# spcl/EBCC

Measured on AMD Instinct MI355X. Metric: fp32 GB/s encode+decode, 721x1440 ERA5 frames MAX_ERROR=0.5, higher is better.
Workload: dtype f32; 1 GPU; 256-frame batch 721x1440 fp32 per GPU, base_cr=30 MAX_ERROR=0.5 (BASELINE configs[1]); frames_per_gpu=256, parallelism=frames sharded over 1 GPU(s), no collective, hw_queues=4, encode_slices=3

## Files before the change

### ebcc_amd/csrc/engine.hip

```cpp
#include "engine.hpp"

#include <algorithm>
#include <atomic>
#include <cstdarg>
#include <mutex>
#include <string>
#include <type_traits>
#include <cstring>
#include <vector>

#include "../../include/ebcc_hip.h"
#include "search.hpp"

namespace ebcc {

static thread_local std::string g_last_error;

void set_error(const char *fmt, ...)
{
    char buf[512];
    va_list ap;
    va_start(ap, fmt);
    vsnprintf(buf, sizeof buf, fmt, ap);
    va_end(ap);
// ... 583 lines not shown
        EBCC_HIP_CHECK(hipMemcpyAsync(ctx->d_u64b, ctx->h_u64b, n_frames * sizeof(unsigned long long), hipMemcpyHostToDevice, s));
        EBCC_HIP_CHECK(hipMemcpyAsync(ctx->d_active, ctx->h_active, n_frames * sizeof(int), hipMemcpyHostToDevice, s));
        launch_prefix_synthesis_stats(d_data, d_decoded, ctx->rb, (int) n_frames, ctx->d_u64b, ctx->d_active, s);
        fetch_frame_states(ctx, n_frames);
        for (size_t f = 0; f < n_frames; f++) { maxerr_bits[f] = ctx->h_fs[f].maxerr_bits; err_sum[f] = ctx->h_fs[f].err_sum; }
        for (size_t f = 0; f < n_frames; f++) ctx->h_fs[f].exit_above = 0.0f;
        push_frame_states(ctx, n_frames);
        wait_stream(s);
        return 0;
    }
    if (!ensure_cut_slots(ctx, (int) n_probes)) { set_error("ebcc_hip_residual_probe: no cut slots for %zu probes of this grid", n_probes); return 1; }
    const CutSlots &cs = ctx->cut;
    std::vector<FrameState> vfs(n_probes);
    std::vector<unsigned long long> bits(n_probes);
    std::vector<int> on(n_probes), of(n_probes);
    for (size_t v = 0; v < n_probes; v++) {
        bits[v] = cut_bits[v]; on[v] = active[v] ? 1 : 0; of[v] = frame_of[v];
        vfs[v] = ctx->h_fs[frame_of[v]];
        vfs[v].exit_above = exit_above[v];
        vfs[v].maxerr_bits = maxerr_bits[v]; vfs[v].err_sum = err_sum[v];
    }
    EBCC_HIP_CHECK(hipMemcpyAsync(cs.fs, vfs.data(), n_probes * sizeof(FrameState), hipMemcpyHostToDevice, s));
    EBCC_HIP_CHECK(hipMemcpyAsync(cs.bits, bits.data(), n_probes * sizeof(unsigned long long), hipMemcpyHostToDevice, s));
    EBCC_HIP_CHECK(hipMemcpyAsync(cs.active, on.data(), n_probes * sizeof(int), hipMemcpyHostToDevice, s));
    EBCC_HIP_CHECK(hipMemcpyAsync(cs.frame_of, of.data(), n_probes * sizeof(int), hipMemcpyHostToDevice, s));
    launch_prefix_synthesis_slots(d_data, d_decoded, ctx->rb, cs, (int) n_probes, s);
    EBCC_HIP_CHECK(hipMemcpyAsync(vfs.data(), cs.fs, n_probes * sizeof(FrameState), hipMemcpyDeviceToHost, s));
    wait_stream(s);
    for (size_t v = 0; v < n_probes; v++) { maxerr_bits[v] = vfs[v].maxerr_bits; err_sum[v] = vfs[v].err_sum; }
    return 0;
    EBCC_API_CATCH(1)
}

}
int ebcc::check_ims_header(ebcc_hip_ctx *ctx, const uint8_t *b, size_t n, size_t num_bits)
{
    if (n < 15 || b[0] != 'I' || b[1] != 'M' || b[2] != 'S') { set_error("SPIHT stream: bad magic"); return 1; }
    unsigned long long hi = 0;
    for (int i = 0; i < 8; i++) hi = (hi << 8) | b[3 + i];
    unsigned lo = ((unsigned) b[11] << 8) | b[12];
    unsigned stages = (unsigned) (hi >> 58), sx = (unsigned) (hi >> 46) & 0xFFF, sy = (unsigned) (hi >> 34) & 0xFFF;
    unsigned ex = (unsigned) (hi >> 24) & 0x3FF, ey = (unsigned) (hi >> 14) & 0x3FF;
    unsigned long long bits0 = ((hi & 0x1FFF) << 16) | lo;
    const Grid &g = ctx->rb.g;
    if ((int) stages != g.stages || (int) sx != g.size_x || (int) sy != g.size_y || (int) ex != g.extra_x ||
        (int) ey != g.extra_y) {
        set_error("SPIHT stream geometry (%u stages, %ux%u +%u,%u) does not match the context (%dx%d)", stages, sx, sy,
                  ex, ey, g.size_x, g.size_y);
        return 1;
    }
    unsigned long long nb = num_bits > bits0 ? bits0 : num_bits;
    if (nb <= 128) { set_error("SPIHT stream: num_bits must exceed 128"); return 1; }
    return 0;
}
extern "C" {

int ebcc_hip_spiht_decode(ebcc_hip_ctx *ctx, const uint8_t *const *streams, const size_t *sizes,
                          const size_t *num_bits, size_t n_frames, float *d_images_out)
{
    EBCC_API_TRY
    if (check_batch(ctx, n_frames, "ebcc_hip_spiht_decode")) return 1;
    hipStream_t s = ctx->stream;
    const size_t slot = ctx->rb.stream_words * 4;
    for (size_t f = 0; f < n_frames; f++) {
        if (sizes[f] > slot - 64) { set_error("SPIHT stream of %zu bytes exceeds the slot", sizes[f]); return 1; }
        if (check_ims_header(ctx, streams[f], sizes[f], num_bits[f])) return 1;
// ... 16 lines not shown
```

### ebcc_amd/csrc/residual.hpp

```cpp
#pragma once

#include "common.hpp"

namespace ebcc {

struct FrameState {
    unsigned long long min_key, max_key;
    float minv, maxv;
    int has_nonfinite;
    int const_field;
    unsigned long long rmin_key, rmax_key;
    float rmin, rmax;
    double dc_sum;
    float dc;
    int dc_uncertain;
    int cmax;
    int top_step;
    unsigned long long budget;
    unsigned long long emitted;
    unsigned int stream_bytes;
    unsigned int refine_base[32];
    unsigned int refine_count[32];
    unsigned int step_reached[32];
    unsigned int maxerr_bits;
    double err_sum;
    unsigned long long nbad;
    float exit_above;
    int dec_stages, dec_dc, dec_top_step;
    unsigned long long dec_budget;
};

struct ResidualBuffers {
    Grid g;
    int max_frames;
    size_t np;
    float *A, *T;
    int32_t *C;
    int32_t *D, *G;
    uint32_t *lip, *lsp, *lis0, *lis1;
    uint32_t *sigord, *lspidx;
    uint32_t *stream;
    size_t stream_words;
    double *partial;
    FrameState *fs;
};
constexpr int kPartials = 256;

struct CutSlots {
    int capacity = 0;
    size_t stride = 0;
    float *A = nullptr, *T = nullptr, *D = nullptr;
    FrameState *fs = nullptr;
    double *partial = nullptr;
    unsigned long long *bits = nullptr;
    int *active = nullptr;
    int *frame_of = nullptr;
};
bool prefix_slots_supported(const ResidualBuffers &rb, int n_slots);
void launch_slots_setup(const ResidualBuffers &rb, const CutSlots &cs, int n_slots, hipStream_t s);
void launch_prefix_synthesis_slots(const float *data, const float *decoded, const ResidualBuffers &rb, const CutSlots &cs, int n_slots, hipStream_t s);
// ... 48 lines not shown
```

### ebcc_amd/csrc/residual_device.hpp

```cpp
#pragma once

#include "residual.hpp"

namespace ebcc {

__device__ inline float prefix_value_of(uint32_t o, int c, uint32_t slot, unsigned long long B, const unsigned int *rbase, const unsigned int *rreach)
{
    float out = 0.0f;
    if (o != 0xFFFFFFFFu && (unsigned long long) o <= B) {
        const unsigned int a = (unsigned int) (c < 0 ? -c : c);
        const int ss = 31 - __clz(a);
        unsigned int mag = 1u << ss;
        for (int s = ss - 1; s >= 0; --s) {
            if (!rreach[s]) break;
            const unsigned long long ord = (unsigned long long) rbase[s] + slot + 1;
            if (ord > B + 1) break;
            mag |= a & (1u << s);
        }
        out = c < 0 ? -(float) mag : (float) mag;
    }
    return out;
}
__device__ inline float prefix_value(const int32_t *__restrict__ C, const uint32_t *__restrict__ so, const uint32_t *__restrict__ li, size_t i,
                                     unsigned long long B, const unsigned int *rbase, const unsigned int *rreach)
{
    const uint32_t o = so[i];
    if (o == 0xFFFFFFFFu || (unsigned long long) o > B) return 0.0f;
    return prefix_value_of(o, C[i], li[i], B, rbase, rreach);
}

}
```

### ebcc_amd/csrc/residual_dwt.hip

```cpp
#include <cstring>
#include <cmath>
#include <mutex>
#include "residual.hpp"
#include "residual_device.hpp"
#include "j2k.hpp"

namespace ebcc {

namespace {

__device__ constexpr float kAlpha = -1.586134342f;
__device__ constexpr float kBeta  = -0.05298011854f;
__device__ constexpr float kGamma = 0.8829110762f;
__device__ constexpr float kDelta = 0.44355068522f;
__device__ constexpr float kXi    = 1.149604398f;

constexpr int kRowThreads = 256;
constexpr int kColThreads = 1024;

template <typename Idx>
__device__ inline void lift_forward_tile(float *E, float *O, int half, int lines, Idx at, int tid, int nt)
{
    const int total = half * lines;
    for (int i = tid; i < total; i += nt) {
        int k = i / lines, l = i - k * lines;
        float o = O[at(k, l)];
        if (k + 1 < half) o = o + kAlpha * (E[at(k, l)] + E[at(k + 1, l)]);
        else              o = o + (2 * kAlpha) * E[at(k, l)];
        O[at(k, l)] = o;
    }
    __syncthreads();
    for (int i = tid; i < total; i += nt) {
        int k = i / lines, l = i - k * lines;
        float e = E[at(k, l)];
        if (k > 0) e = e + kBeta * (O[at(k, l)] + O[at(k - 1, l)]);
// ... 345 lines not shown
    {
        const float E0 = div_xi(Ein), O0 = Oin * kXi;
        int k = j - 1;
        float e1 = 0;
        if (k >= 0 && k < half) e1 = E_1 - kDelta * (O_1 + (k > 0 ? O_2 : O0));
        k = j - 2;
        float o1 = 0;
        if (k >= 0 && k < half) o1 = O_2 - kGamma * (a1 + (k + 1 < half ? e1 : a2));
        k = j - 3;
        float e2 = 0;
        if (k >= 0 && k < half) e2 = a2 - kBeta * (b1 + (k > 0 ? b2 : o1));
        k = j - 4;
        x_even = c1;
        x_odd = (k + 1 < half) ? b2 - kAlpha * (c1 + e2) : b2 - (2 * kAlpha) * c1;
        O_2 = O_1; O_1 = O0; E_1 = E0;
        a2 = a1; a1 = e1;
        b2 = b1; b1 = o1;
        c1 = e2;
    }
    __device__ void interior(float Ein, float Oin, float &x_even, float &x_odd)
    {
        const float E0 = div_xi(Ein), O0 = Oin * kXi;
        const float e1 = E_1 - kDelta * (O_1 + O_2);
        const float o1 = O_2 - kGamma * (a1 + e1);
        const float e2 = a2 - kBeta * (b1 + b2);
        x_even = c1;
        x_odd = b2 - kAlpha * (c1 + e2);
        O_2 = O_1; O_1 = O0; E_1 = E0;
        a2 = a1; a1 = e1;
        b2 = b1; b1 = o1;
        c1 = e2;
    }
};

constexpr int kStreamT = 128;
__global__ __launch_bounds__(kStreamT) void k_cols_inv_stream(const float *__restrict__ src, float *__restrict__ dst, Grid g, size_t np,
                                                               const int32_t *__restrict__ Cb, const uint32_t *__restrict__ sigordb,
                                                               const uint32_t *__restrict__ lspidxb, const FrameState *fsb,
                                                               const unsigned long long *trunc_bits, const int *active)
{
    const int frame = blockIdx.y;
    if (active && !active[frame]) return;
    const FrameState &fs = fsb[frame];
    unsigned long long nb = trunc_bits[frame], bits0 = fs.budget + 128;
    if (nb > bits0) nb = bits0;
    const unsigned long long B = nb - 128;
    __shared__ unsigned int rbase[32], rreach[32];
    if (threadIdx.x < 32) { rbase[threadIdx.x] = fs.refine_base[threadIdx.x]; rreach[threadIdx.x] = fs.step_reached[threadIdx.x]; }
    __syncthreads();
    const int nx = g.nx, ny = g.ny, half = ny >> 1, hx = nx >> 1;
    const int col = blockIdx.x * kStreamT + threadIdx.x;
    if (col >= nx) return;
    const float *a = src + (size_t) frame * np;
    float *out = dst + (size_t) frame * np;
    const int32_t *C = Cb + (size_t) frame * np;
    const uint32_t *so = sigordb + (size_t) frame * np, *li = lspidxb + (size_t) frame * np;
    const int per = (half + (int) gridDim.z - 1) / (int) gridDim.z, ka = (int) blockIdx.z * per, kb = min(half, ka + per);
    const int jstart = max(ka - 2, 0);
    struct Raw { float ll; uint32_t eo, el; int ec; uint32_t oo, ol; int oc; };
    const bool left = col < hx;
    auto fetch = [&](int j, Raw &r) {
        const int jj = min(j, half - 1);
        const size_t ie = (size_t) jj * nx + col, io = (size_t) (half + jj) * nx + col;
        r.ll = left ? a[ie] : 0.0f;
        r.eo = left ? 0xFFFFFFFFu : so[ie]; r.ec = 0; r.el = 0;
        if (r.eo != 0xFFFFFFFFu && (unsigned long long) r.eo <= B) { r.ec = C[ie]; r.el = li[ie]; }
        r.oo = so[io]; r.oc = 0; r.ol = 0;
        if (r.oo != 0xFFFFFFFFu && (unsigned long long) r.oo <= B) { r.oc = C[io]; r.ol = li[io]; }
    };
    auto value = [&](const Raw &r, float &e, float &o) {
        e = left ? r.ll : prefix_value_of(r.eo, r.ec, r.el, B, rbase, rreach);
        o = prefix_value_of(r.oo, r.oc, r.ol, B, rbase, rreach);
    };
    RPipe p;
    Raw cur;
    fetch(jstart, cur);
    for (int j = jstart; j < kb + 4; j++) {
        Raw nxt;
        fetch(j + 1, nxt);
        float e_in, o_in, xe, xo;
        value(cur, e_in, o_in);
        p.step(j, half, e_in, o_in, xe, xo);
        const int k = j - 4;
        if (k >= ka && k < kb) {
            out[(size_t) (2 * k) * nx + col] = xe;
            out[(size_t) (2 * k + 1) * nx + col] = xo;
        }
        cur = nxt;
    }
}

constexpr int kFusePairs = 60;
constexpr int kFuseMaxWaves = 16;
__global__ __launch_bounds__(64 * kFuseMaxWaves) void k_finest_inv_use(const float *__restrict__ src, Grid g, size_t np, const int32_t *__restrict__ Cb,
                                                        const uint32_t *__restrict__ sigordb, const uint32_t *__restrict__ lspidxb,
                                                        const unsigned long long *trunc_bits, const int *active, RowUse u, int strips, int n_frames, int pieces,
                                                        const int *frame_of, size_t src_stride)
{
    struct { int strip, frame, piece; } tb{(int) blockIdx.x * ((int) blockDim.x >> 6) + ((int) threadIdx.x >> 6), (int) blockIdx.y % n_frames, (int) blockIdx.y / n_frames};
    const int slot = tb.frame;
    if (active && !active[slot]) return;
    const int frame = frame_of ? frame_of[slot] : slot;
    const FrameState &fs = u.fs[slot];
    unsigned long long nb = trunc_bits[slot], bits0 = fs.budget + 128;
    if (nb > bits0) nb = bits0;
    const unsigned long long B = nb - 128;
    __shared__ unsigned int rbase[32], rreach[32];
    if (threadIdx.x < 32) { rbase[threadIdx.x] = fs.refine_base[threadIdx.x]; rreach[threadIdx.x] = fs.step_reached[threadIdx.x]; }
    __syncthreads();
    if (tb.strip >= strips) return;
    const int lane = (int) threadIdx.x & 63;
    const int nx = g.nx, ny = g.ny, half = ny >> 1, hx = nx >> 1;
    const int k = tb.strip * kFusePairs + lane - 2;
    const bool in_range = k >= 0 && k < hx;
    const bool owner = lane >= 2 && lane < 2 + kFusePairs && in_range;
    const int kc = min(max(k, 0), hx - 1);
    const float *a = src + (size_t) slot * src_stride;
    const int32_t *C = Cb + (size_t) frame * np;
    const uint32_t *so = sigordb + (size_t) frame * np, *li = lspidxb + (size_t) frame * np;
    const float *x = u.data + (size_t) frame * u.n_pix, *d = u.decoded + (size_t) frame * u.n_pix;
    const float dc = fs.dc, rmin = fs.rmin, rng = fs.rmax - fs.rmin;
    const int per = (half + pieces - 1) / pieces, ka = tb.piece * per, kb = min(half, ka + per);
    const size_t part = (size_t) slot * kPartials + (size_t) (tb.strip + strips * tb.piece);
    const int jstart = max(ka - 2, 0);
    const float exit_above = fs.exit_above;
    if (exit_above > 0.0f && __uint_as_float(__hip_atomic_load(&u.fs[slot].maxerr_bits, __ATOMIC_RELAXED, __HIP_MEMORY_SCOPE_AGENT)) > exit_above) {
        if (lane == 0) u.partial[part] = 0.0;
        return;
    }
    struct Det { uint32_t o, l; int c; };
    struct Raw { float ll; Det lh, hl, hh; };
    auto det = [&](size_t i, Det &t) {
        t.o = so[i]; t.c = 0; t.l = 0;
        if (t.o != 0xFFFFFFFFu && (unsigned long long) t.o <= B) { t.c = C[i]; t.l = li[i]; }
    };
    auto fetch = [&](int j, Raw &r) {
        const int jj = min(j, half - 1);
        const size_t top = (size_t) jj * nx, bot = (size_t) (half + jj) * nx;
        r.ll = a[top + kc];
        det(bot + kc, r.lh);
        det(top + hx + kc, r.hl);
        det(bot + hx + kc, r.hh);
    };
    auto val = [&](const Det &t) { return prefix_value_of(t.o, t.c, t.l, B, rbase, rreach); };
    const bool first = !(k > 0), last = !(k + 1 < hx);
    auto hsynth = [&](float e_raw, float o_raw, float &even, float &odd) {
        const float E0 = div_xi(e_raw), O0 = o_raw * kXi;
        const float Ol = lane_below(O0), Or = lane_above(O0);
        const float e1 = E0 - kDelta * (O0 + (first ? Or : Ol));
        const float e1l = lane_below(e1), e1r = lane_above(e1);
        const float o1 = O0 - kGamma * (e1 + (last ? e1l : e1r));
        const float o1l = lane_below(o1), o1r = lane_above(o1);
        const float e2 = e1 - kBeta * (o1 + (first ? o1r : o1l));
        const float e2r = lane_above(e2);
        even = e2;
        odd = last ? o1 - (2 * kAlpha) * e2 : o1 - kAlpha * (e2 + e2r);
    };
    double acc = 0;
    float mx = 0;
    auto use_row = [&](bool mine, int y, float s0, float s1, float x0, float x1, float d0, float d1) {
        const bool m0 = mine && y < u.size_y && 2 * k < u.size_x, m1 = mine && y < u.size_y && 2 * k + 1 < u.size_x;
        const float t0 = x0 - (d0 + residual_value_fast(s0, dc, rmin, rng)), t1 = x1 - (d1 + residual_value_fast(s1, dc, rmin, rng));
        acc += m0 ? (double) t0 : 0.0;
        acc += m1 ? (double) t1 : 0.0;
        mx = m0 ? fmaxf(mx, fabsf(t0)) : mx;
        mx = m1 ? fmaxf(mx, fabsf(t1)) : mx;
    };
    RPipe pl, ph;
    Raw cur;
    fetch(jstart, cur);
    const int c0 = min(2 * kc, u.size_x - 1), c1 = min(2 * kc + 1, u.size_x - 1);
    typedef float f32x2 __attribute__((ext_vector_type(2)));
    const bool pair_io = (u.size_x & 1) == 0 && (u.n_pix & 1) == 0 && (((size_t) x | (size_t) d) & 7) == 0;
    const unsigned cp = 2u * (unsigned) min(kc, max((u.size_x >> 1) - 1, 0));
    for (int j = jstart; j < kb + 4; j++) {
        Raw nxt;
        fetch(j + 1, nxt);
        const int kk = j - 4;
        const unsigned y0 = (unsigned) min(max(2 * kk, 0), u.size_y - 1), y1 = (unsigned) min(max(2 * kk + 1, 0), u.size_y - 1);
        float x00, x01, x10, x11, d00, d01, d10, d11;
        if (pair_io) {
            const unsigned i0 = y0 * (unsigned) u.size_x + cp, i1 = y1 * (unsigned) u.size_x + cp;
            const f32x2 xa = *reinterpret_cast<const f32x2 *>(x + i0), xb = *reinterpret_cast<const f32x2 *>(x + i1);
            const f32x2 da = *reinterpret_cast<const f32x2 *>(d + i0), db = *reinterpret_cast<const f32x2 *>(d + i1);
            x00 = xa.x; x01 = xa.y; x10 = xb.x; x11 = xb.y; d00 = da.x; d01 = da.y; d10 = db.x; d11 = db.y;
        } else {
            const unsigned i00 = y0 * (unsigned) u.size_x + c0, i01 = y0 * (unsigned) u.size_x + c1, i10 = y1 * (unsigned) u.size_x + c0, i11 = y1 * (unsigned) u.size_x + c1;
            x00 = x[i00]; x01 = x[i01]; x10 = x[i10]; x11 = x[i11]; d00 = d[i00]; d01 = d[i01]; d10 = d[i10]; d11 = d[i11];
        }
        float le, lo, he, ho;
        if (j >= 4 && j < half) {
            pl.interior(cur.ll, val(cur.lh), le, lo);
            ph.interior(val(cur.hl), val(cur.hh), he, ho);
        } else {
            pl.step(j, half, cur.ll, val(cur.lh), le, lo);
            ph.step(j, half, val(cur.hl), val(cur.hh), he, ho);
        }
        const bool mine = owner && kk >= ka && kk < kb;
        if (kk >= ka) {
            float s00, s01, s10, s11;
            hsynth(le, he, s00, s01);
            hsynth(lo, ho, s10, s11);
            use_row(mine, 2 * kk, s00, s01, x00, x01, d00, d01);
            use_row(mine, 2 * kk + 1, s10, s11, x10, x11, d10, d11);
        }
        cur = nxt;
    }
    for (int q = 32; q >= 1; q >>= 1) { acc += __shfl_xor(acc, q); mx = fmaxf(mx, __shfl_xor(mx, q)); }
    if (lane == 0) {
        u.partial[part] = acc;
        atomicMax(&u.fs[slot].maxerr_bits, __float_as_uint(mx));
    }
}

__global__ __launch_bounds__(64) void k_level_inv_fused(const float *__restrict__ ll, const float *__restrict__ det, float *__restrict__ dst,
                                                         int stride, size_t np, int nx, int ny, const int *active, int strips, int n_frames, int pieces)
{
    const int strip = (int) blockIdx.x, frame = (int) blockIdx.y % n_frames, piece = (int) blockIdx.y / n_frames;
    if (active && !active[frame]) return;
    const int lane = (int) threadIdx.x;
    const int half = ny >> 1, hx = nx >> 1;
    const int k = strip * kFusePairs + lane - 2;
    const bool owner = lane >= 2 && lane < 2 + kFusePairs && k >= 0 && k < hx;
    const int kc = min(max(k, 0), hx - 1);
    const float *a = ll + (size_t) frame * np, *b = det + (size_t) frame * np;
    float *out = dst + (size_t) frame * np;
    const int per = (half + pieces - 1) / pieces, ka = piece * per, kb = min(half, ka + per);
    if (ka >= kb) return;
    const int jstart = max(ka - 2, 0);
    struct Raw { float ll, lh, hl, hh; };
    auto fetch = [&](int j, Raw &r) {
        const int jj = min(j, half - 1);
        const size_t top = (size_t) jj * stride, bot = (size_t) (half + jj) * stride;
        r.ll = a[top + kc];
        r.lh = b[bot + kc];
        r.hl = b[top + hx + kc];
        r.hh = b[bot + hx + kc];
    };
    const bool first = !(k > 0), last = !(k + 1 < hx);
    auto hsynth = [&](float e_raw, float o_raw, float &even, float &odd) {
        const float E0 = div_xi(e_raw), O0 = o_raw * kXi;
        const float Ol = lane_below(O0), Or = lane_above(O0);
        const float e1 = E0 - kDelta * (O0 + (first ? Or : Ol));
        const float e1l = lane_below(e1), e1r = lane_above(e1);
        const float o1 = O0 - kGamma * (e1 + (last ? e1l : e1r));
        const float o1l = lane_below(o1), o1r = lane_above(o1);
        const float e2 = e1 - kBeta * (o1 + (first ? o1r : o1l));
        const float e2r = lane_above(e2);
        even = e2;
        odd = last ? o1 - (2 * kAlpha) * e2 : o1 - kAlpha * (e2 + e2r);
    };
    RPipe pl, ph;
    Raw cur;
    fetch(jstart, cur);
    for (int j = jstart; j < kb + 4; j++) {
        Raw nxt;
        fetch(j + 1, nxt);
        const int kk = j - 4;
        float le, lo, he, ho;
        if (j >= 4 && j < half) {
            pl.interior(cur.ll, cur.lh, le, lo);
            ph.interior(cur.hl, cur.hh, he, ho);
        } else {
            pl.step(j, half, cur.ll, cur.lh, le, lo);
            ph.step(j, half, cur.hl, cur.hh, he, ho);
        }
        if (kk >= ka) {
            float s00, s01, s10, s11;
            hsynth(le, he, s00, s01);
            hsynth(lo, ho, s10, s11);
            if (owner && kk < kb) {
                *reinterpret_cast<float2 *>(out + (size_t) (2 * kk) * stride + 2 * k) = make_float2(s00, s01);
                *reinterpret_cast<float2 *>(out + (size_t) (2 * kk + 1) * stride + 2 * k) = make_float2(s10, s11);
            }
        }
        cur = nxt;
    }
}

__global__ void k_minmax_init(FrameState *fs, int n_frames)
{
    int f = blockIdx.x * blockDim.x + threadIdx.x;
    if (f < n_frames) {
        fs[f].rmin_key = ~0ull;
        fs[f].rmax_key = 0ull;
    }
}

__device__ inline unsigned long long wave_min_u64(unsigned long long v)
{
    for (int d = 32; d >= 1; d >>= 1) {
        unsigned long long o = __shfl_xor(v, d);
        v = o < v ? o : v;
    }
    return v;
}
__device__ inline unsigned long long wave_max_u64(unsigned long long v)
{
    for (int d = 32; d >= 1; d >>= 1) {
        unsigned long long o = __shfl_xor(v, d);
        v = o > v ? o : v;
    }
    return v;
// ... 407 lines not shown
    const float *fine_ll = rb.A;
    const bool finest_fused = ceil_div(g.nx >> 1, kFusePairs) * 8 <= kPartials && (g.nx >> 1) >= 2;
    if (finest_fused && (long long) n_frames * 8 <= 65535) {
        float *scratch[2] = {rb.T, reinterpret_cast<float *>(rb.D)};
        const float *ll = rb.A;
        int turn = 0;
        for (int lv = g.stages - 1; lv >= 1; lv--) {
            const int nx = g.nx >> lv, ny = g.ny >> lv;
            const int lstrips = ceil_div(nx >> 1, kFusePairs), lpieces = std::max(1, std::min(8, (ny >> 1) / 16));
            hipLaunchKernelGGL(k_level_inv_fused, dim3((unsigned) lstrips, (unsigned) (n_frames * lpieces)), dim3(64), 0, s, ll, rb.A, scratch[turn], g.nx, rb.np,
                               nx, ny, d_active, lstrips, n_frames, lpieces);
            ll = scratch[turn];
            turn ^= 1;
        }
        fine_ll = ll;
    } else {
        for (int lv = g.stages - 1; lv >= 1; lv--) {
            int nx = g.nx >> lv, ny = g.ny >> lv;
            cols_pass<false>(rb.A, rb.T, rb, ny, nx, n_frames, d_active, s);
            rows_inv(rb.T, rb.A, rb, nx, ny, n_frames, d_active, s);
        }
    }
    int pieces = std::max(1, std::min(8, (g.ny >> 1) / 16));
    while (pieces > 1 && (long long) n_frames * pieces > 65535) pieces--;
    RowUse u{};
    u.data = data; u.decoded = decoded;
    int partials;
    const int strips = ceil_div(g.nx >> 1, kFusePairs);
    if (strips * pieces <= kPartials && (g.nx >> 1) >= 2) {
        u.size_x = g.size_x; u.size_y = g.size_y; u.n_pix = (size_t) g.size_x * g.size_y; u.fs = rb.fs; u.partial = rb.partial;
        const int wave_cap = 1;
        const int wg = std::min(strips, wave_cap);
        hipLaunchKernelGGL(k_finest_inv_use, dim3((unsigned) ceil_div(strips, wg), (unsigned) (n_frames * pieces)), dim3(64 * wg), 0, s, fine_ll, g, rb.np, rb.C, rb.sigord, rb.lspidx,
                           d_trunc_bits, d_active, u, strips, n_frames, pieces, (const int *) nullptr, rb.np);
        partials = strips * pieces;
    } else {
        hipLaunchKernelGGL(k_cols_inv_stream, dim3(ceil_div(g.nx, kStreamT), n_frames, pieces), dim3(kStreamT), 0, s, rb.A, rb.T, g, rb.np, rb.C,
                           rb.sigord, rb.lspidx, rb.fs, d_trunc_bits, d_active);
        partials = synthesis_tail(rb, n_frames, d_active, s, u);
    }
    hipLaunchKernelGGL(k_probe_finish, dim3(ceil_div(n_frames, 64)), dim3(64), 0, s, rb.partial, partials, rb.fs, n_frames, d_active);
    EBCC_HIP_LAUNCH_CHECK();
}

__global__ void k_residual_budget(FrameState *fs, const unsigned long long *bits0, int n_frames, const int *active)
{
    const int f = blockIdx.x * blockDim.x + threadIdx.x;
    if (f >= n_frames || (active && !active[f])) return;
    fs[f].budget = bits0[f] - 128;
    fs[f].exit_above = 0.0f;
}
__global__ void k_whole_stream_cut(FrameState *fs, unsigned long long *trunc_bits, int n_frames, const int *active)
{
    const int f = blockIdx.x * blockDim.x + threadIdx.x;
    if (f >= n_frames || (active && !active[f])) return;
    trunc_bits[f] = (unsigned long long) fs[f].stream_bytes * 8ull;
    fs[f].dec_dc = (int) fs[f].dc;
}
void launch_residual_budget(const ResidualBuffers &rb, int n_frames, const unsigned long long *d_bits0, const int *d_active, hipStream_t s)
{
    hipLaunchKernelGGL(k_residual_budget, dim3(ceil_div(n_frames, 64)), dim3(64), 0, s, rb.fs, d_bits0, n_frames, d_active);
    EBCC_HIP_LAUNCH_CHECK();
}
void launch_whole_stream_cut(const ResidualBuffers &rb, int n_frames, unsigned long long *d_trunc_bits, const int *d_active, hipStream_t s)
{
    hipLaunchKernelGGL(k_whole_stream_cut, dim3(ceil_div(n_frames, 64)), dim3(64), 0, s, rb.fs, d_trunc_bits, n_frames, d_active);
    EBCC_HIP_LAUNCH_CHECK();
}

void launch_reconstruct_coarse_slots(const ResidualBuffers &rb, const CutSlots &cs, int n_slots, hipStream_t s);
__global__ void k_slots_setup(FrameState *vfs, const FrameState *fs, const int *frame_of, int n_slots)
{
    const int v = blockIdx.x * blockDim.x + threadIdx.x;
    if (v < n_slots) vfs[v] = fs[frame_of[v]];
}
bool prefix_slots_supported(const ResidualBuffers &rb, int n_slots)
{
    const Grid &g = rb.g;
    if (g.stages < 2 || g.ny < 32 || (g.nx >> 1) < 2) return false;
    const int pieces = std::max(1, std::min(8, (g.ny >> 1) / 16));
    return ceil_div(g.nx >> 1, kFusePairs) * 8 <= kPartials && (long long) n_slots * 8 <= 65535 && ceil_div(g.nx >> 1, kFusePairs) * pieces <= kPartials;
}
void launch_slots_setup(const ResidualBuffers &rb, const CutSlots &cs, int n_slots, hipStream_t s)
{
    hipLaunchKernelGGL(k_slots_setup, dim3(ceil_div(n_slots, 64)), dim3(64), 0, s, cs.fs, rb.fs, cs.frame_of, n_slots);
    EBCC_HIP_LAUNCH_CHECK();
}
void launch_prefix_synthesis_slots(const float *data, const float *decoded, const ResidualBuffers &rb, const CutSlots &cs, int n_slots, hipStream_t s)
{
    const Grid &g = rb.g;
    hipLaunchKernelGGL(k_probe_init, dim3(ceil_div(n_slots, 64)), dim3(64), 0, s, cs.fs, n_slots, cs.active);
    launch_reconstruct_coarse_slots(rb, cs, n_slots, s);
    float *scratch[2] = {cs.T, cs.D};
    const float *ll = cs.A;
    int turn = 0;
    for (int lv = g.stages - 1; lv >= 1; lv--) {
        const int nx = g.nx >> lv, ny = g.ny >> lv;
        const int lstrips = ceil_div(nx >> 1, kFusePairs), lpieces = std::max(1, std::min(8, (ny >> 1) / 16));
        hipLaunchKernelGGL(k_level_inv_fused, dim3((unsigned) lstrips, (unsigned) (n_slots * lpieces)), dim3(64), 0, s, ll, cs.A, scratch[turn], g.nx, cs.stride,
                           nx, ny, cs.active, lstrips, n_slots, lpieces);
        ll = scratch[turn];
        turn ^= 1;
    }
    int pieces = std::max(1, std::min(8, (g.ny >> 1) / 16));
    while (pieces > 1 && (long long) n_slots * pieces > 65535) pieces--;
    RowUse u{};
    u.data = data; u.decoded = decoded;
    u.size_x = g.size_x; u.size_y = g.size_y; u.n_pix = (size_t) g.size_x * g.size_y; u.fs = cs.fs; u.partial = cs.partial;
    const int strips = ceil_div(g.nx >> 1, kFusePairs);
    hipLaunchKernelGGL(k_finest_inv_use, dim3((unsigned) strips, (unsigned) (n_slots * pieces)), dim3(64), 0, s, ll, g, rb.np, rb.C, rb.sigord, rb.lspidx,
                       cs.bits, cs.active, u, strips, n_slots, pieces, cs.frame_of, cs.stride);
    hipLaunchKernelGGL(k_probe_finish, dim3(ceil_div(n_slots, 64)), dim3(64), 0, s, cs.partial, strips * pieces, cs.fs, n_slots, cs.active);
    EBCC_HIP_LAUNCH_CHECK();
}

void launch_synthesis_tail_add(float *out, const ResidualBuffers &rb, int n_frames, const int *d_active, hipStream_t s, int row0, int col0,
                               int rows, int cols)
{
    const Grid &g = rb.g;
    hipLaunchKernelGGL(k_rows_inv_add, dim3(min(rows, 96), n_frames), dim3(kRowThreads), (size_t) g.nx * sizeof(float), s, rb.T, g.nx, rb.np, g.nx,
                       d_active, rb.fs, out, row0, col0, rows, cols);
    EBCC_HIP_LAUNCH_CHECK();
}

void launch_synthesis_tail_add_placed(float *out, const ResidualBuffers &rb, const J2kBoxEntry *d_boxes, const J2kPlacement *d_places, size_t n_boxes,
                                      const int *d_active, hipStream_t s, int max_rows)
{
    const Grid &g = rb.g;
    for (size_t lo = 0; lo < n_boxes; lo += 65535) {
        const unsigned n = (unsigned) std::min<size_t>(65535, n_boxes - lo);
        hipLaunchKernelGGL(k_rows_inv_add_placed, dim3(min(max_rows, 96), n), dim3(kRowThreads), (size_t) g.nx * sizeof(float), s, rb.T, g.nx, rb.np,
                           g.nx, d_active, rb.fs, out, d_boxes + lo, d_places + lo);
    }
    EBCC_HIP_LAUNCH_CHECK();
}

void launch_emit_image(float *image_out, const ResidualBuffers &rb, int n_frames, hipStream_t s)
{
    size_t n_pix = (size_t) rb.g.size_x * rb.g.size_y;
    hipLaunchKernelGGL(k_emit_image, dim3(128, n_frames), dim3(256), 0, s, image_out, rb.A, rb.g, n_pix, rb.np, rb.fs);
    EBCC_HIP_LAUNCH_CHECK();
}

int residual_selfcheck_divisions()
// ... 15 lines not shown
```

### include/ebcc_hip.h

```cpp
#ifndef EBCC_HIP_H
#define EBCC_HIP_H

#include <stddef.h>
#include <stdint.h>

#include "ebcc_codec.h"

#ifdef __cplusplus
extern "C" {
#endif
#pragma GCC visibility push(default)

typedef struct ebcc_hip_ctx ebcc_hip_ctx;

int ebcc_hip_device_count(void);
#define EBCC_HIP_MAX_FRAMES 65535
ebcc_hip_ctx *ebcc_hip_create(int device, size_t max_frames, size_t height, size_t width);
void ebcc_hip_destroy(ebcc_hip_ctx *ctx);
void *ebcc_hip_stream(ebcc_hip_ctx *ctx);
size_t ebcc_hip_workspace_bytes(const ebcc_hip_ctx *ctx);

void *ebcc_hip_malloc(size_t bytes);
void ebcc_hip_free(void *d_ptr);
int ebcc_hip_memcpy_h2d(void *d_dst, const void *src, size_t bytes);
int ebcc_hip_memcpy_d2h(void *dst, const void *d_src, size_t bytes);


int ebcc_hip_spiht_encode(ebcc_hip_ctx *ctx, const float *d_images, size_t n_frames, const size_t *trunc_bits,
                          uint8_t **out_streams, size_t *out_sizes);

int ebcc_hip_spiht_decode(ebcc_hip_ctx *ctx, const uint8_t *const *streams, const size_t *sizes,
                          const size_t *num_bits, size_t n_frames, float *d_images_out);

int ebcc_hip_spiht_decode_prefix(ebcc_hip_ctx *ctx, size_t n_frames, const size_t *trunc_bits, float *d_images_out);

int ebcc_hip_spiht_coeffs(ebcc_hip_ctx *ctx, const float *d_images, size_t n_frames, int32_t *coeffs, int *dc);
size_t ebcc_hip_padded_pixels(const ebcc_hip_ctx *ctx);

int ebcc_hip_residual_prepare(ebcc_hip_ctx *ctx, const float *d_data, const float *d_decoded, size_t n_frames, const size_t *budget_bits,
                              float *rmin, float *rmax, int *dc, uint8_t **out_streams, size_t *out_sizes);
int ebcc_hip_residual_probe(ebcc_hip_ctx *ctx, const float *d_data, const float *d_decoded, size_t n_frames, int slots, size_t n_probes,
                            const int *frame_of, const size_t *cut_bits, const int *active, const float *exit_above,
                            uint32_t *maxerr_bits, double *err_sum);

int ebcc_hip_j2k_encode(ebcc_hip_ctx *ctx, const float *d_frames, size_t n_frames, const float *cr, uint8_t **out_streams,
                        size_t *out_sizes, float *minmax);
int ebcc_hip_j2k_emulated_decode(ebcc_hip_ctx *ctx, const float *d_frames, size_t n_frames, const float *target,
                                 float *d_out, unsigned long long *nbad, double *err_sum);
int ebcc_hip_j2k_probe(ebcc_hip_ctx *ctx, const float *d_frames, size_t n_frames, const float *cr, const float *target,
                       const uint32_t *bad_limit, const int *keep, const int *active, int keep_field, unsigned long long *nbad,
                       double *err_sum, int *stream_bytes, float *d_field_out);
int ebcc_hip_j2k_decode(ebcc_hip_ctx *ctx, const uint8_t *const *streams, const size_t *sizes, size_t n_frames,
                        const float *minmax, float *d_out);

int ebcc_hip_j2k_parse_check(const uint8_t *cs, size_t n, size_t height, size_t width);

int ebcc_hip_prepare(ebcc_hip_ctx *ctx, size_t n_frames);
void ebcc_hip_release_engines(void);
void ebcc_hip_release_second_set(ebcc_hip_ctx *ctx);
int ebcc_hip_upload(ebcc_hip_ctx *ctx, void *d_dst, const void *h_src, size_t bytes);
int ebcc_hip_download(ebcc_hip_ctx *ctx, void *h_dst, const void *d_src, size_t bytes);
int ebcc_hip_encode_host_frames(ebcc_hip_ctx *ctx, const float *h_frames, size_t n_frames, const codec_config_t *config,
                                uint8_t **out_streams, size_t *out_sizes);
int ebcc_hip_decode_host_frames(ebcc_hip_ctx *ctx, const uint8_t *const *streams, const size_t *sizes, size_t n_frames,
                                float *h_frames_out);
int ebcc_hip_prefault(void *h_dst, size_t bytes);
int ebcc_hip_encode_frames(ebcc_hip_ctx *ctx, const float *d_frames, size_t n_frames, const codec_config_t *config,
                           uint8_t **out_streams, size_t *out_sizes);
int ebcc_hip_decode_frames(ebcc_hip_ctx *ctx, const uint8_t *const *streams, const size_t *sizes, size_t n_frames,
                           float *d_frames_out);
int ebcc_hip_encode_shard(ebcc_hip_ctx *ctx, const float *d_frames, size_t n_frames, const codec_config_t *config,
                          uint8_t **out_streams, size_t *out_sizes);
int ebcc_hip_decode_shard(ebcc_hip_ctx *ctx, const uint8_t *const *streams, const size_t *sizes, size_t n_frames,
                          float *d_frames_out);


// ... 147 lines not shown
```

Baseline: 9.050 GB/s.

## Add early-exit polling and violating-tile hints to residual probe kernel

```diff
diff --git a/ebcc_amd/csrc/engine.hip b/ebcc_amd/csrc/engine.hip
--- a/ebcc_amd/csrc/engine.hip
+++ b/ebcc_amd/csrc/engine.hip
@@ -639,6 +639,21 @@
     EBCC_API_CATCH(1)
 }
 
+int ebcc_hip_residual_hint(ebcc_hip_ctx *ctx, size_t frame, int set_tile, int *tile)
+{
+    EBCC_API_TRY
+    if (check_batch(ctx, frame + 1, "ebcc_hip_residual_hint")) return 1;
+    hipStream_t s = ctx->stream;
+    int *d_hint = &ctx->rb.fs[frame].probe_hint;
+    if (set_tile >= 0) EBCC_HIP_CHECK(hipMemcpyAsync(d_hint, &set_tile, sizeof(int), hipMemcpyHostToDevice, s));
+    int now = 0;
+    EBCC_HIP_CHECK(hipMemcpyAsync(&now, d_hint, sizeof(int), hipMemcpyDeviceToHost, s));
+    wait_stream(s);
+    if (tile) *tile = now;
+    return 0;
+    EBCC_API_CATCH(1)
+}
+
 }
 int ebcc::check_ims_header(ebcc_hip_ctx *ctx, const uint8_t *b, size_t n, size_t num_bits)
 {
diff --git a/ebcc_amd/csrc/residual.hpp b/ebcc_amd/csrc/residual.hpp
--- a/ebcc_amd/csrc/residual.hpp
+++ b/ebcc_amd/csrc/residual.hpp
@@ -26,6 +26,7 @@
     double err_sum;
     unsigned long long nbad;
     float exit_above;
+    int probe_hint;
     int dec_stages, dec_dc, dec_top_step;
     unsigned long long dec_budget;
 };
diff --git a/ebcc_amd/csrc/residual_device.hpp b/ebcc_amd/csrc/residual_device.hpp
--- a/ebcc_amd/csrc/residual_device.hpp
+++ b/ebcc_amd/csrc/residual_device.hpp
@@ -4,23 +4,26 @@
 
 namespace ebcc {
 
+__device__ inline float prefix_value_inside(int c, uint32_t slot, unsigned long long B, const unsigned int *rbase, const unsigned int *rreach)
+{
+    const unsigned int a = (unsigned int) (c < 0 ? -c : c);
+    const int ss = 31 - __clz(a);
+    unsigned int mag = 1u << ss;
+    for (int s = ss - 1; s >= 0; --s) {
+        if (!rreach[s]) break;
+        const unsigned long long ord = (unsigned long long) rbase[s] + slot + 1;
+        if (ord > B + 1) break;
+        mag |= a & (1u << s);
+    }
+    return c < 0 ? -(float) mag : (float) mag;
+}
 __device__ inline float prefix_value_of(uint32_t o, int c, uint32_t slot, unsigned long long B, const unsigned int *rbase, const unsigned int *rreach)
 {
     float out = 0.0f;
-    if (o != 0xFFFFFFFFu && (unsigned long long) o <= B) {
-        const unsigned int a = (unsigned int) (c < 0 ? -c : c);
-        const int ss = 31 - __clz(a);
-        unsigned int mag = 1u << ss;
-        for (int s = ss - 1; s >= 0; --s) {
-            if (!rreach[s]) break;
-            const unsigned long long ord = (unsigned long long) rbase[s] + slot + 1;
-            if (ord > B + 1) break;
-            mag |= a & (1u << s);
-        }
-        out = c < 0 ? -(float) mag : (float) mag;
-    }
+    if (o != 0xFFFFFFFFu && (unsigned long long) o <= B) out = prefix_value_inside(c, slot, B, rbase, rreach);
     return out;
 }
+__device__ inline uint32_t prefix_cut32(unsigned long long B) { return B < 0xFFFFFFFEull ? (uint32_t) B : 0xFFFFFFFEu; }
 __device__ inline float prefix_value(const int32_t *__restrict__ C, const uint32_t *__restrict__ so, const uint32_t *__restrict__ li, size_t i,
                                      unsigned long long B, const unsigned int *rbase, const unsigned int *rreach)
 {
diff --git a/ebcc_amd/csrc/residual_dwt.hip b/ebcc_amd/csrc/residual_dwt.hip
--- a/ebcc_amd/csrc/residual_dwt.hip
+++ b/ebcc_amd/csrc/residual_dwt.hip
@@ -1,6 +1,7 @@
 #include <cstring>
 #include <cmath>
 #include <mutex>
+#include <type_traits>
 #include "residual.hpp"
 #include "residual_device.hpp"
 #include "j2k.hpp"
@@ -412,6 +413,23 @@
         c1 = e2;
     }
 };
+
+template <bool kEdge>
+__device__ __forceinline__ void hsynth_pair(bool first, bool last, float e_raw, float o_raw, float &even, float &odd)
+{
+    const float E0 = div_xi(e_raw), O0 = o_raw * kXi;
+    const float Ol = lane_below(O0), Or = lane_above(O0);
+    const float e1 = E0 - kDelta * (O0 + (kEdge && first ? Or : Ol));
+    const float e1l = lane_below(e1), e1r = lane_above(e1);
+    const float o1 = O0 - kGamma * (e1 + (kEdge && last ? e1l : e1r));
+    const float o1l = lane_below(o1), o1r = lane_above(o1);
+    const float e2 = e1 - kBeta * (o1 + (kEdge && first ? o1r : o1l));
+    const float e2r = lane_above(e2);
+    even = e2;
+    odd = kEdge && last ? o1 - (2 * kAlpha) * e2 : o1 - kAlpha * (e2 + e2r);
+}
+constexpr int kFusePairs = 60;
+__device__ inline bool strip_has_row_end(int strip, int hx) { return strip == 0 || strip * kFusePairs + 62 >= hx; }
 
 constexpr int kStreamT = 128;
 __global__ __launch_bounds__(kStreamT) void k_cols_inv_stream(const float *__restrict__ src, float *__restrict__ dst, Grid g, size_t np,
@@ -470,12 +488,16 @@
     }
 }
 
-constexpr int kFusePairs = 60;
 constexpr int kFuseMaxWaves = 16;
+#ifndef EBCC_PROBE_POLL_STEPS
+#define EBCC_PROBE_POLL_STEPS 4
+#endif
+constexpr int kPollSteps = EBCC_PROBE_POLL_STEPS;
+static_assert(kPollSteps > 0 && (kPollSteps & (kPollSteps - 1)) == 0, "a power of two");
 __global__ __launch_bounds__(64 * kFuseMaxWaves) void k_finest_inv_use(const float *__restrict__ src, Grid g, size_t np, const int32_t *__restrict__ Cb,
                                                         const uint32_t *__restrict__ sigordb, const uint32_t *__restrict__ lspidxb,
                                                         const unsigned long long *trunc_bits, const int *active, RowUse u, int strips, int n_frames, int pieces,
-                                                        const int *frame_of, size_t src_stride)
+                                                        const int *frame_of, size_t src_stride, FrameState *frame_fs)
 {
     struct { int strip, frame, piece; } tb{(int) blockIdx.x * ((int) blockDim.x >> 6) + ((int) threadIdx.x >> 6), (int) blockIdx.y % n_frames, (int) blockIdx.y / n_frames};
     const int slot = tb.frame;
@@ -485,10 +507,19 @@
     unsigned long long nb = trunc_bits[slot], bits0 = fs.budget + 128;
     if (nb > bits0) nb = bits0;
     const unsigned long long B = nb - 128;
+    const uint32_t Bc = prefix_cut32(B);
     __shared__ unsigned int rbase[32], rreach[32];
     if (threadIdx.x < 32) { rbase[threadIdx.x] = fs.refine_base[threadIdx.x]; rreach[threadIdx.x] = fs.step_reached[threadIdx.x]; }
     __syncthreads();
     if (tb.strip >= strips) return;
+    const float exit_above = fs.exit_above;
+    if (exit_above > 0.0f) {
+        const int hint = fs.probe_hint;
+        if ((unsigned) hint < (unsigned) (strips * pieces)) {
+            tb.strip = (tb.strip + hint % strips) % strips;
+            tb.piece = (tb.piece + hint / strips) % pieces;
+        }
+    }
     const int lane = (int) threadIdx.x & 63;
     const int nx = g.nx, ny = g.ny, half = ny >> 1, hx = nx >> 1;
     const int k = tb.strip * kFusePairs + lane - 2;
@@ -503,16 +534,19 @@
     const int per = (half + pieces - 1) / pieces, ka = tb.piece * per, kb = min(half, ka + per);
     const size_t part = (size_t) slot * kPartials + (size_t) (tb.strip + strips * tb.piece);
     const int jstart = max(ka - 2, 0);
-    const float exit_above = fs.exit_above;
-    if (exit_above > 0.0f && __uint_as_float(__hip_atomic_load(&u.fs[slot].maxerr_bits, __ATOMIC_RELAXED, __HIP_MEMORY_SCOPE_AGENT)) > exit_above) {
-        if (lane == 0) u.partial[part] = 0.0;
-        return;
+    unsigned int seen = 0;
+    if (exit_above > 0.0f) {
+        seen = __hip_atomic_load(&u.fs[slot].maxerr_bits, __ATOMIC_RELAXED, __HIP_MEMORY_SCOPE_AGENT);
+        if (__uint_as_float(seen) > exit_above) {
+            if (lane == 0) u.partial[part] = 0.0;
+            return;
+        }
     }
     struct Det { uint32_t o, l; int c; };
     struct Raw { float ll; Det lh, hl, hh; };
     auto det = [&](size_t i, Det &t) {
         t.o = so[i]; t.c = 0; t.l = 0;
-        if (t.o != 0xFFFFFFFFu && (unsigned long long) t.o <= B) { t.c = C[i]; t.l = li[i]; }
+        if (t.o <= Bc) { t.c = C[i]; t.l = li[i]; }
     };
     auto fetch = [&](int j, Raw &r) {
         const int jj = min(j, half - 1);
@@ -522,24 +556,14 @@
         det(top + hx + kc, r.hl);
         det(bot + hx + kc, r.hh);
     };
-    auto val = [&](const Det &t) { return prefix_value_of(t.o, t.c, t.l, B, rbase, rreach); };
+    auto val = [&](const Det &t) { return t.o <= Bc ? prefix_value_inside(t.c, t.l, B, rbase, rreach) : 0.0f; };
     const bool first = !(k > 0), last = !(k + 1 < hx);
-    auto hsynth = [&](float e_raw, float o_raw, float &even, float &odd) {
-        const float E0 = div_xi(e_raw), O0 = o_raw * kXi;
-        const float Ol = lane_below(O0), Or = lane_above(O0);
-        const float e1 = E0 - kDelta * (O0 + (first ? Or : Ol));
-        const float e1l = lane_below(e1), e1r = lane_above(e1);
-        const float o1 = O0 - kGamma * (e1 + (last ? e1l : e1r));
-        const float o1l = lane_below(o1), o1r = lane_above(o1);
-        const float e2 = e1 - kBeta * (o1 + (first ? o1r : o1l));
-        const float e2r = lane_above(e2);
-        even = e2;
-        odd = last ? o1 - (2 * kAlpha) * e2 : o1 - kAlpha * (e2 + e2r);
-    };
+    const bool row_end = strip_has_row_end(tb.strip, hx);
     double acc = 0;
     float mx = 0;
-    auto use_row = [&](bool mine, int y, float s0, float s1, float x0, float x1, float d0, float d1) {
-        const bool m0 = mine && y < u.size_y && 2 * k < u.size_x, m1 = mine && y < u.size_y && 2 * k + 1 < u.size_x;
+    const bool own0 = owner && 2 * k < u.size_x, own1 = owner && 2 * k + 1 < u.size_x;
+    auto use_row = [&](bool row_in, float s0, float s1, float x0, float x1, float d0, float d1) {
+        const bool m0 = own0 && row_in, m1 = own1 && row_in;
         const float t0 = x0 - (d0 + residual_value_fast(s0, dc, rmin, rng)), t1 = x1 - (d1 + residual_value_fast(s1, dc, rmin, rng));
         acc += m0 ? (double) t0 : 0.0;
         acc += m1 ? (double) t1 : 0.0;
@@ -553,43 +577,70 @@
     typedef float f32x2 __attribute__((ext_vector_type(2)));
     const bool pair_io = (u.size_x & 1) == 0 && (u.n_pix & 1) == 0 && (((size_t) x | (size_t) d) & 7) == 0;
     const unsigned cp = 2u * (unsigned) min(kc, max((u.size_x >> 1) - 1, 0));
-    for (int j = jstart; j < kb + 4; j++) {
-        Raw nxt;
-        fetch(j + 1, nxt);
-        const int kk = j - 4;
-        const unsigned y0 = (unsigned) min(max(2 * kk, 0), u.size_y - 1), y1 = (unsigned) min(max(2 * kk + 1, 0), u.size_y - 1);
-        float x00, x01, x10, x11, d00, d01, d10, d11;
-        if (pair_io) {
-            const unsigned i0 = y0 * (unsigned) u.size_x + cp, i1 = y1 * (unsigned) u.size_x + cp;
-            const f32x2 xa = *reinterpret_cast<const f32x2 *>(x + i0), xb = *reinterpret_cast<const f32x2 *>(x + i1);
-            const f32x2 da = *reinterpret_cast<const f32x2 *>(d + i0), db = *reinterpret_cast<const f32x2 *>(d + i1);
-            x00 = xa.x; x01 = xa.y; x10 = xb.x; x11 = xb.y; d00 = da.x; d01 = da.y; d10 = db.x; d11 = db.y;
-        } else {
-            const unsigned i00 = y0 * (unsigned) u.size_x + c0, i01 = y0 * (unsigned) u.size_x + c1, i10 = y1 * (unsigned) u.size_x + c0, i11 = y1 * (unsigned) u.size_x + c1;
-            x00 = x[i00]; x01 = x[i01]; x10 = x[i10]; x11 = x[i11]; d00 = d[i00]; d01 = d[i01]; d10 = d[i10]; d11 = d[i11];
-        }
-        float le, lo, he, ho;
-        if (j >= 4 && j < half) {
-            pl.interior(cur.ll, val(cur.lh), le, lo);
-            ph.interior(val(cur.hl), val(cur.hh), he, ho);
-        } else {
-            pl.step(j, half, cur.ll, val(cur.lh), le, lo);
-            ph.step(j, half, val(cur.hl), val(cur.hh), he, ho);
-        }
-        const bool mine = owner && kk >= ka && kk < kb;
-        if (kk >= ka) {
-            float s00, s01, s10, s11;
-            hsynth(le, he, s00, s01);
-            hsynth(lo, ho, s10, s11);
-            use_row(mine, 2 * kk, s00, s01, x00, x01, d00, d01);
-            use_row(mine, 2 * kk + 1, s10, s11, x10, x11, d10, d11);
-        }
-        cur = nxt;
+    auto run = [&](auto poll) -> bool {
+        for (int j = jstart; j < kb + 4; j++) {
+            Raw nxt;
+            fetch(j + 1, nxt);
+            const int kk = j - 4;
+            const unsigned y0 = (unsigned) min(max(2 * kk, 0), u.size_y - 1), y1 = (unsigned) min(max(2 * kk + 1, 0), u.size_y - 1);
+            float x00, x01, x10, x11, d00, d01, d10, d11;
+            if (pair_io) {
+                const unsigned i0 = y0 * (unsigned) u.size_x + cp, i1 = y1 * (unsigned) u.size_x + cp;
+                const f32x2 xa = *reinterpret_cast<const f32x2 *>(x + i0), xb = *reinterpret_cast<const f32x2 *>(x + i1);
+                const f32x2 da = *reinterpret_cast<const f32x2 *>(d + i0), db = *reinterpret_cast<const f32x2 *>(d + i1);
+                x00 = xa.x; x01 = xa.y; x10 = xb.x; x11 = xb.y; d00 = da.x; d01 = da.y; d10 = db.x; d11 = db.y;
+            } else {
+                const unsigned i00 = y0 * (unsigned) u.size_x + c0, i01 = y0 * (unsigned) u.size_x + c1, i10 = y1 * (unsigned) u.size_x + c0, i11 = y1 * (unsigned) u.size_x + c1;
+                x00 = x[i00]; x01 = x[i01]; x10 = x[i10]; x11 = x[i11]; d00 = d[i00]; d01 = d[i01]; d10 = d[i10]; d11 = d[i11];
+            }
+            float le, lo, he, ho;
+            if (j >= 4 && j < half) {
+                pl.interior(cur.ll, val(cur.lh), le, lo);
+                ph.interior(val(cur.hl), val(cur.hh), he, ho);
+            } else {
+                pl.step(j, half, cur.ll, val(cur.lh), le, lo);
+                ph.step(j, half, val(cur.hl), val(cur.hh), he, ho);
+            }
+            if (kk >= ka) {
+                float s00, s01, s10, s11;
+                if (row_end) {
+                    hsynth_pair<true>(first, last, le, he, s00, s01);
+                    hsynth_pair<true>(first, last, lo, ho, s10, s11);
+                } else {
+                    hsynth_pair<false>(false, false, le, he, s00, s01);
+                    hsynth_pair<false>(false, false, lo, ho, s10, s11);
+                }
+                const bool rows_in = kk < kb;
+                use_row(rows_in && 2 * kk < u.size_y, s00, s01, x00, x01, d00, d01);
+                use_row(rows_in && 2 * kk + 1 < u.size_y, s10, s11, x10, x11, d10, d11);
+            }
+            cur = nxt;
+            if constexpr (decltype(poll)::value) {
+                if (((j - jstart) & (kPollSteps - 1)) == kPollSteps - 1) {
+                    if (__any(mx > exit_above) || __uint_as_float(seen) > exit_above) return true;
+                    seen = __hip_atomic_load(&u.fs[slot].maxerr_bits, __ATOMIC_RELAXED, __HIP_MEMORY_SCOPE_AGENT);
+                }
+            }
+        }
+        return false;
+    };
+    const int tile = tb.strip + strips * tb.piece;
+    if (exit_above > 0.0f ? run(std::true_type{}) : run(std::false_type{})) {
+        for (int q = 32; q >= 1; q >>= 1) mx = fmaxf(mx, __shfl_xor(mx, q));
+        if (lane == 0) {
+            if (mx > exit_above) {
+                atomicMax(&u.fs[slot].maxerr_bits, __float_as_uint(mx));
+                frame_fs[frame].probe_hint = tile;
+            }
+            u.partial[part] = 0.0;
+        }
+        return;
     }
     for (int q = 32; q >= 1; q >>= 1) { acc += __shfl_xor(acc, q); mx = fmaxf(mx, __shfl_xor(mx, q)); }
     if (lane == 0) {
         u.partial[part] = acc;
         atomicMax(&u.fs[slot].maxerr_bits, __float_as_uint(mx));
+        if (exit_above > 0.0f && mx > exit_above) frame_fs[frame].probe_hint = tile;
     }
 }
 
@@ -618,18 +669,7 @@
         r.hh = b[bot + hx + kc];
     };
     const bool first = !(k > 0), last = !(k + 1 < hx);
-    auto hsynth = [&](float e_raw, float o_raw, float &even, float &odd) {
-        const float E0 = div_xi(e_raw), O0 = o_raw * kXi;
-        const float Ol = lane_below(O0), Or = lane_above(O0);
-        const float e1 = E0 - kDelta * (O0 + (first ? Or : Ol));
-        const float e1l = lane_below(e1), e1r = lane_above(e1);
-        const float o1 = O0 - kGamma * (e1 + (last ? e1l : e1r));
-        const float o1l = lane_below(o1), o1r = lane_above(o1);
-        const float e2 = e1 - kBeta * (o1 + (first ? o1r : o1l));
-        const float e2r = lane_above(e2);
-        even = e2;
-        odd = last ? o1 - (2 * kAlpha) * e2 : o1 - kAlpha * (e2 + e2r);
-    };
+    const bool row_end = strip_has_row_end(strip, hx);
     RPipe pl, ph;
     Raw cur;
     fetch(jstart, cur);
@@ -647,8 +687,13 @@
         }
         if (kk >= ka) {
             float s00, s01, s10, s11;
-            hsynth(le, he, s00, s01);
-            hsynth(lo, ho, s10, s11);
+            if (row_end) {
+                hsynth_pair<true>(first, last, le, he, s00, s01);
+                hsynth_pair<true>(first, last, lo, ho, s10, s11);
+            } else {
+                hsynth_pair<false>(false, false, le, he, s00, s01);
+                hsynth_pair<false>(false, false, lo, ho, s10, s11);
+            }
             if (owner && kk < kb) {
                 *reinterpret_cast<float2 *>(out + (size_t) (2 * kk) * stride + 2 * k) = make_float2(s00, s01);
                 *reinterpret_cast<float2 *>(out + (size_t) (2 * kk + 1) * stride + 2 * k) = make_float2(s10, s11);
@@ -1122,7 +1167,7 @@
         const int wave_cap = 1;
         const int wg = std::min(strips, wave_cap);
         hipLaunchKernelGGL(k_finest_inv_use, dim3((unsigned) ceil_div(strips, wg), (unsigned) (n_frames * pieces)), dim3(64 * wg), 0, s, fine_ll, g, rb.np, rb.C, rb.sigord, rb.lspidx,
-                           d_trunc_bits, d_active, u, strips, n_frames, pieces, (const int *) nullptr, rb.np);
+                           d_trunc_bits, d_active, u, strips, n_frames, pieces, (const int *) nullptr, rb.np, rb.fs);
         partials = strips * pieces;
     } else {
         hipLaunchKernelGGL(k_cols_inv_stream, dim3(ceil_div(g.nx, kStreamT), n_frames, pieces), dim3(kStreamT), 0, s, rb.A, rb.T, g, rb.np, rb.C,
@@ -1139,6 +1184,7 @@
     if (f >= n_frames || (active && !active[f])) return;
     fs[f].budget = bits0[f] - 128;
     fs[f].exit_above = 0.0f;
+    fs[f].probe_hint = 0;
 }
 __global__ void k_whole_stream_cut(FrameState *fs, unsigned long long *trunc_bits, int n_frames, const int *active)
 {
@@ -1199,7 +1245,7 @@
     u.size_x = g.size_x; u.size_y = g.size_y; u.n_pix = (size_t) g.size_x * g.size_y; u.fs = cs.fs; u.partial = cs.partial;
     const int strips = ceil_div(g.nx >> 1, kFusePairs);
     hipLaunchKernelGGL(k_finest_inv_use, dim3((unsigned) strips, (unsigned) (n_slots * pieces)), dim3(64), 0, s, ll, g, rb.np, rb.C, rb.sigord, rb.lspidx,
-                       cs.bits, cs.active, u, strips, n_slots, pieces, cs.frame_of, cs.stride);
+                       cs.bits, cs.active, u, strips, n_slots, pieces, cs.frame_of, cs.stride, rb.fs);
     hipLaunchKernelGGL(k_probe_finish, dim3(ceil_div(n_slots, 64)), dim3(64), 0, s, cs.partial, strips * pieces, cs.fs, n_slots, cs.active);
     EBCC_HIP_LAUNCH_CHECK();
 }
diff --git a/include/ebcc_hip.h b/include/ebcc_hip.h
--- a/include/ebcc_hip.h
+++ b/include/ebcc_hip.h
@@ -42,6 +42,7 @@
 int ebcc_hip_residual_probe(ebcc_hip_ctx *ctx, const float *d_data, const float *d_decoded, size_t n_frames, int slots, size_t n_probes,
                             const int *frame_of, const size_t *cut_bits, const int *active, const float *exit_above,
                             uint32_t *maxerr_bits, double *err_sum);
+int ebcc_hip_residual_hint(ebcc_hip_ctx *ctx, size_t frame, int set_tile, int *tile);
 
 int ebcc_hip_j2k_encode(ebcc_hip_ctx *ctx, const float *d_frames, size_t n_frames, const float *cr, uint8_t **out_streams,
                         size_t *out_sizes, float *minmax);
```

Result: no change. 9.016 GB/s (-0.4%).
